# openjamoses/TOSEM-2021-Replication

Measured on AMD Instinct MI355X. Metric: train_tokens_per_s, higher is better.
Workload: dtype bf16; 1 GPU; model=mltc-base, global_batch=128, seq_len=512, parallelism=dp1

## Files before the change

csrc/flash_attn.hip:

```cpp

#include "common.h"
#include "launchers.h"
#include "philox.h"

typedef __attribute__((ext_vector_type(16))) float f32x16;
typedef __attribute__((ext_vector_type(2))) unsigned uint2_t;
typedef __attribute__((ext_vector_type(4))) unsigned uint4_t;

#define FA_DH 64
#define FA_KVB 32
#define FA_QB 32
#define FA_WAVES 4
#define FA_BLOCK (FA_WAVES * WAVE)
#define FA_QWG (FA_WAVES * FA_QB)
#define FA_Q2WG (2 * FA_QWG)

#define TILE_LDS_BYTES (FA_KVB * 128)
#define FWD_LDS_BYTES (2 * TILE_LDS_BYTES + FA_WAVES * 64 * sizeof(float))
#define BWD_LDS_BYTES (2 * TILE_LDS_BYTES + 64 * sizeof(float))
#define BWD_SEG_LDS_BYTES (BWD_LDS_BYTES + 32 * sizeof(int))
#define DQ_LDS_BYTES TILE_LDS_BYTES
#define DQR_LDS_BYTES (2 * TILE_LDS_BYTES + 16)
#define FA_DQR_WAVES(drop) ((drop) ? 1 : 2)

struct FaGeom {
  long qkv_bs, qkv_hs; int qkv_rs;
  long o_bs, o_hs; int o_rs;
  static FaGeom bhld(int H, int L) {
    return {(long)H * L * FA_DH, (long)L * FA_DH, FA_DH,
            (long)H * L * FA_DH, (long)L * FA_DH, FA_DH};
  }
  static FaGeom packed(int H, int L) {
    const int D = H * FA_DH;
    return {(long)L * 3 * D, 64L, 3 * D, (long)L * D, 64L, D};
  }
};


__device__ __forceinline__ int kswz(int row, int byte_off) {
  return byte_off ^ ((row & 7) << 4);
}

__device__ __forceinline__ int c_row(int r, int half) {
  return (r & 3) + 8 * (r >> 2) + 4 * half;
}

struct FaStager {
  int row, byte;
  __device__ __forceinline__ explicit FaStager(int tid)
      : row(tid >> 3), byte((tid & 7) * 16) {}
  __device__ __forceinline__ short8_t load(const short* base, int row0,
                                           int rs) const {
    return *(const short8_t*)(base + (long)(row0 + row) * rs + (byte >> 1));
  }
  __device__ __forceinline__ void store(short* lds, short8_t v) const {
    *(short8_t*)((char*)lds + row * 128 + kswz(row, byte)) = v;
  }
};

__device__ __forceinline__ short8_t tile_row_frag(const short* lds, int col,
                                                  int half, int c) {
  return *(const short8_t*)((const char*)lds + col * 128 +
                            kswz(col, (16 * c + 8 * half) * 2));
}

__device__ __forceinline__ void cvt_pk_swap(const float (&s)[16], int r0,
                                            int r1, uint4_t& u, int i) {
  unsigned lo, hi;
  asm("v_cvt_pk_bf16_f32 %0, %1, %2\n\ts_nop 1" : "=v"(lo)
      : "v"(s[r0]), "v"(s[r0 + 1]));
  asm("v_cvt_pk_bf16_f32 %0, %1, %2\n\ts_nop 1" : "=v"(hi)
      : "v"(s[r1]), "v"(s[r1 + 1]));
  auto sw = __builtin_amdgcn_permlane32_swap(lo, hi, false, false);
  u[i] = sw[0]; u[i + 2] = sw[1];
}

__device__ __forceinline__ void c_to_afrag2(const float (&sa)[16],
                                            short8_t (&fa)[2],
                                            const float (&sb)[16],
                                            short8_t (&fb)[2]) {
#pragma unroll
  for (int c = 0; c < 2; ++c) {
    uint4_t ua, ub;
#pragma unroll
    for (int i = 0; i < 2; ++i) {
      int r0 = c * 8 + 2 * i;
      int r1 = c * 8 + 4 + 2 * i;
      cvt_pk_swap(sa, r0, r1, ua, i);
      cvt_pk_swap(sb, r0, r1, ub, i);
    }
    fa[c] = __builtin_bit_cast(short8_t, ua);
    fb[c] = __builtin_bit_cast(short8_t, ub);
  }
}

struct FaTrFrags {
  uint2_t r[8];
  __device__ __forceinline__ short8_t frag(int c, int t) const {
    uint4_t w;
    w[0] = r[c * 4 + 0 * 2 + t][0];
    w[1] = r[c * 4 + 0 * 2 + t][1];
    w[2] = r[c * 4 + 1 * 2 + t][0];
    w[3] = r[c * 4 + 1 * 2 + t][1];
    return __builtin_bit_cast(short8_t, w);
  }
};

struct FaTrOffsets { unsigned a[8]; };

__device__ __forceinline__ FaTrOffsets tr_offsets(int lane, int half) {
  const int row_mate = (lane >> 2) & 3;
  const int d_lane = 16 * ((lane >> 4) & 1) + 4 * (lane & 3);
  FaTrOffsets o;
#pragma unroll
  for (int c = 0; c < 2; ++c)
#pragma unroll
    for (int rr = 0; rr < 2; ++rr)
#pragma unroll
      for (int t = 0; t < 2; ++t) {
        int row = 16 * c + 8 * half + 4 * rr + row_mate;
        int dcol = (32 * t + d_lane) * 2;
        o.a[c * 4 + rr * 2 + t] = row * 128 + kswz(row, dcol);
      }
  return o;
}

__device__ __forceinline__ void tr_issue(const short* lds,
                                         const FaTrOffsets& o, FaTrFrags& f) {
  const unsigned base = (unsigned)(unsigned long)(char*)lds;
  unsigned a[8];
#pragma unroll
  for (int i = 0; i < 8; ++i) a[i] = base + o.a[i];
  asm volatile(
      "ds_read_b64_tr_b16 %0, %8\n\t"
      "ds_read_b64_tr_b16 %1, %9\n\t"
      "ds_read_b64_tr_b16 %2, %10\n\t"
      "ds_read_b64_tr_b16 %3, %11\n\t"
      "ds_read_b64_tr_b16 %4, %12\n\t"
      "ds_read_b64_tr_b16 %5, %13\n\t"
      "ds_read_b64_tr_b16 %6, %14\n\t"
      "ds_read_b64_tr_b16 %7, %15\n\t"
      "s_waitcnt lgkmcnt(0)"
      : "=&v"(f.r[0]), "=&v"(f.r[1]), "=&v"(f.r[2]), "=&v"(f.r[3]),
        "=&v"(f.r[4]), "=&v"(f.r[5]), "=&v"(f.r[6]), "=&v"(f.r[7])
      : "v"(a[0]), "v"(a[1]), "v"(a[2]), "v"(a[3]), "v"(a[4]), "v"(a[5]),
        "v"(a[6]), "v"(a[7])
      : "memory");
}

__device__ __forceinline__ void tr_gather(const short* lds,
                                          const FaTrOffsets& o, FaTrFrags& f) {
  tr_issue(lds, o, f);
  __builtin_amdgcn_sched_barrier(0);
}

struct FaQBlocks { int bh, qA, qB; };

__device__ __forceinline__ FaQBlocks fa_qblocks(int L, int wid) {
  const int n_qblocks = (L + FA_Q2WG - 1) / FA_Q2WG;
  const int bid = xcd_group_remap(blockIdx.x, gridDim.x, n_qblocks);
  const int qA = (bid % n_qblocks) * FA_Q2WG + wid * FA_QB;
  return {bid / n_qblocks, qA, qA + FA_QWG};
}

__device__ __forceinline__ float fa_half_merge(float s) {
  return s + __shfl_xor(s, 32, WAVE);
}

__device__ __forceinline__ void fa_colsum_merge_store(const float* cs, int tid,
                                                      float* dst0,
                                                      float* dst1) {
  if (tid < 2 * FA_DH) {
    const int slot = tid / FA_DH, c = tid % FA_DH;
    const float* p = cs + slot * FA_WAVES * FA_DH + c;
    float s = p[0];
#pragma unroll
    for (int w = 1; w < FA_WAVES; ++w) s += p[w * FA_DH];
    float* dst = slot ? dst1 : dst0;
    if (dst) dst[c] = s;
  }
}

__device__ __forceinline__ int fa_last_active_kv(const float* mrow, int L,
                                                 int tid, int* scratch) {
  if (tid == 0) *scratch = -1;
  __syncthreads();
  int loc = -1;
  for (int kv = tid; kv < L; kv += FA_BLOCK)
    if (mrow[kv] > -1.0e8f) loc = kv;
  if (loc >= 0) atomicMax(scratch, loc);
  __syncthreads();
  return *scratch;
}

#define FA_SEG_BIAS -1.0e9f

struct FaRange { int lo, hi; };

__device__ __forceinline__ FaRange fa_seg_range(const int* srow, int L,
                                                int r_lo, int r_hi, int tid,
                                                int* scratch) {
  const int s_first = srow[r_lo], s_last = srow[r_hi];
  if (tid == 0) { scratch[0] = r_lo; scratch[1] = r_hi; }
  __syncthreads();
  int lo = r_lo, hi = r_hi;
  for (int j = tid; j < L; j += FA_BLOCK) {
    const int s = srow[j];
    if (s == s_first) lo = min(lo, j);
    if (s == s_last) hi = max(hi, j);
  }
  atomicMin(&scratch[0], lo);
  atomicMax(&scratch[1], hi);
  __syncthreads();
  return {scratch[0], scratch[1]};
}

__device__ __forceinline__ bool fa_seg_tile_live(const int (&r)[16], int a,
                                                 int b) {
  bool hit = false;
#pragma unroll
  for (int i = 0; i < 16; ++i) hit |= (r[i] == a) | (r[i] == b);
  return __builtin_amdgcn_ballot_w64(hit) != 0;
}

__device__ __forceinline__ unsigned long long fa_live_window(
    const unsigned char* dead_bh, int t0, int n_t, int lane) {
  const int t = t0 + lane;
  bool lv = t < n_t;
  if (lv && dead_bh) lv = dead_bh[t] == 0;
  return __builtin_amdgcn_ballot_w64(lv);
}

__device__ __forceinline__ void fa_store_zero_tile(short* base, int rs, int q0,
                                                   int L, int lane) {
#pragma unroll
  for (int i = 0; i < 4; ++i) {
    const int row = q0 + 8 * i + (lane >> 3);
    if (row < L)
      *(short8_t*)(base + (long)row * rs + (lane & 7) * 8) = (short8_t)(0);
  }
}

struct FaLiveScan {
  const unsigned char* dead_bh;
  int n_t, lane, win;
  unsigned long long bits;
  __device__ __forceinline__ FaLiveScan(const unsigned char* d, int n_t_,
                                        int lane_)
      : dead_bh(d), n_t(n_t_), lane(lane_), win(-1), bits(0) {}
  __device__ __forceinline__ void preload() {
    if (dead_bh) { win = 0; bits = fa_live_window(dead_bh, 0, n_t, lane); }
  }
  __device__ __forceinline__ int next(int qt, int n_q) {
    if (!dead_bh) return qt;
    while (qt < n_q) {
      if ((qt >> 6) != win) {
        win = qt >> 6;
        bits = fa_live_window(dead_bh, win << 6, n_t, lane);
      }
      const unsigned long long m = bits >> (qt & 63);
      if (m) return min(qt + (int)__builtin_ctzll(m), n_q);
      qt = (win + 1) << 6;
    }
    return n_q;
  }
};

#ifndef FA_DROP_QUAD_SHARE
#define FA_DROP_QUAD_SHARE 1
#endif

template <int G>
__device__ __forceinline__ unsigned fa_quad_bcast(unsigned v) {
  return (unsigned)__builtin_amdgcn_mov_dpp((int)v, G * 0x55, 0xf, 0xf, true);
}

template <int G>
__device__ __forceinline__ unsigned fa_drop_group_kvreg(const unsigned (&w)[4],
                                                        int i, unsigned thr) {
  const unsigned t0 = fa_quad_bcast<G>(w[0]), t1 = fa_quad_bcast<G>(w[1]);
  const unsigned t2 = fa_quad_bcast<G>(w[2]), t3 = fa_quad_bcast<G>(w[3]);
  const unsigned word = i == 0 ? t0 : i == 1 ? t1 : i == 2 ? t2 : t3;
  unsigned m = 0;
#pragma unroll
  for (int j = 0; j < 4; ++j)
    m |= (((word >> (8 * j)) & 0xffu) >= thr ? 1u : 0u) << (4 * G + j);
  return m;
}

__device__ __forceinline__ unsigned fa_drop_keep16_kvreg(
    const FaDrop& dr, unsigned long long rowblk, int kblk0, int lane) {
  const int i = lane & 3;
  unsigned w[4];
#if FA_DROP_QUAD_SHARE
  fa_drop_block(dr, rowblk + (unsigned)(kblk0 + 2 * i), w);
  return fa_drop_group_kvreg<0>(w, i, dr.thr) |
         fa_drop_group_kvreg<1>(w, i, dr.thr) |
         fa_drop_group_kvreg<2>(w, i, dr.thr) |
         fa_drop_group_kvreg<3>(w, i, dr.thr);
#else
  unsigned m = 0;
#pragma unroll
  for (int g = 0; g < 4; ++g) {
    fa_drop_block(dr, rowblk + (unsigned)(kblk0 + 2 * g), w);
    const unsigned word = i == 0 ? w[0] : i == 1 ? w[1] : i == 2 ? w[2] : w[3];
#pragma unroll
    for (int j = 0; j < 4; ++j)
      m |= (((word >> (8 * j)) & 0xffu) >= dr.thr ? 1u : 0u) << (4 * g + j);
  }
  return m;
#endif
}

template <int G>
__device__ __forceinline__ unsigned fa_drop_group_qreg(const unsigned (&w)[4],
                                                       int sh, unsigned thr) {
  unsigned m = 0;
#pragma unroll
  for (int j = 0; j < 4; ++j)
    m |= (((fa_quad_bcast<G>(w[j]) >> sh) & 0xffu) >= thr ? 1u : 0u)
         << (4 * G + j);
  return m;
}

__device__ __forceinline__ unsigned fa_drop_keep16_qreg(
    const FaDrop& dr, unsigned long long colblk, unsigned nb, int qblk0,
    int lane) {
  const int i = lane & 3;
  unsigned w[4];
#if FA_DROP_QUAD_SHARE
  fa_drop_block(dr, colblk + (unsigned long long)(qblk0 + 2 * i) * nb, w);
  return fa_drop_group_qreg<0>(w, 8 * i, dr.thr) |
         fa_drop_group_qreg<1>(w, 8 * i, dr.thr) |
         fa_drop_group_qreg<2>(w, 8 * i, dr.thr) |
         fa_drop_group_qreg<3>(w, 8 * i, dr.thr);
#else
  unsigned m = 0;
#pragma unroll
  for (int g = 0; g < 4; ++g) {
    fa_drop_block(dr, colblk + (unsigned long long)(qblk0 + 2 * g) * nb, w);
#pragma unroll
    for (int j = 0; j < 4; ++j)
      m |= (((w[j] >> (8 * i)) & 0xffu) >= dr.thr ? 1u : 0u) << (4 * g + j);
  }
  return m;
#endif
}

template <bool SEG, bool DROP>
__global__ void __launch_bounds__(FA_BLOCK, 2)
flash_fwd_kernel(const short* __restrict__ q, const short* __restrict__ k,
                 const short* __restrict__ v, const float* __restrict__ mask,
                 const int* __restrict__ seg,
                 short* __restrict__ o, float* __restrict__ lse,
                 int B, int H, int L, float scale, FaGeom g, FaDrop dr) {
  extern __shared__ __attribute__((aligned(16))) char smem[];
  short* k_lds = (short*)smem;
  short* v_lds = (short*)(smem + TILE_LDS_BYTES);
  float* alpha_lds = (float*)(smem + 2 * TILE_LDS_BYTES);

  const int tid = threadIdx.x;
  const int lane = tid & (WAVE - 1);
  const int wid = tid / WAVE;
  const int col = lane & 31;
  const int half = lane >> 5;
  const FaTrOffsets tro = tr_offsets(lane, half);

  const FaQBlocks qb = fa_qblocks(L, wid);
  const int b = qb.bh / H;
  const int h = qb.bh % H;
  const long qkv_off = (long)b * g.qkv_bs + (long)h * g.qkv_hs;
  const long o_off = (long)b * g.o_bs + (long)h * g.o_hs;
  const int my_qA = qb.qA + col;
  const int my_qB = qb.qB + col;
  const bool validA = my_qA < L;
  const bool validB = my_qB < L;
  const float* mrow = (!SEG && mask) ? mask + (long)b * L : nullptr;
  const int* srow = SEG ? seg + (long)b * L : nullptr;
  int sqA = 0, sqB = 0;
  if constexpr (SEG) {
    sqA = srow[validA ? my_qA : L - 1];
    sqB = srow[validB ? my_qB : L - 1];
  }

  short8_t qfA[4], qfB[4];
  {
    const short* qrA = q + qkv_off + (long)(validA ? my_qA : L - 1) * g.qkv_rs;
    const short* qrB = q + qkv_off + (long)(validB ? my_qB : L - 1) * g.qkv_rs;
#pragma unroll
    for (int c = 0; c < 4; ++c) {
      qfA[c] = *(const short8_t*)(qrA + c * 16 + half * 8);
      qfB[c] = *(const short8_t*)(qrB + c * 16 + half * 8);
    }
  }

  f32x16 oA[2], oB[2];
#pragma unroll
  for (int t = 0; t < 2; ++t) { oA[t] = (f32x16)(0.f); oB[t] = (f32x16)(0.f); }
  float mA = -3.0e38f, lA = 0.f, mB = -3.0e38f, lB = 0.f;
  unsigned long long dblkA = 0, dblkB = 0;
  if constexpr (DROP) {
    const unsigned long long nb = (unsigned)L / 4;
    dblkA = ((unsigned long long)qb.bh * nb + (unsigned)(my_qA >> 2)) * nb;
    dblkB = ((unsigned long long)qb.bh * nb + (unsigned)(my_qB >> 2)) * nb;
  }

  const int n_kv = L / FA_KVB;
  int kt_begin = 0;
  int n_kv_eff = n_kv;
  if (mrow) {
    int last = fa_last_active_kv(mrow, L, tid, (int*)alpha_lds);
    if (last >= 0) n_kv_eff = min(n_kv, last / FA_KVB + 1);
  }
  if constexpr (SEG) {
    const int q_lo = qb.qA - wid * FA_QB;
    const FaRange kr = fa_seg_range(srow, L, q_lo, min(q_lo + FA_Q2WG, L) - 1,
                                    tid, (int*)alpha_lds);
    kt_begin = kr.lo / FA_KVB;
    n_kv_eff = kr.hi / FA_KVB + 1;
  }
  const FaStager st(tid);
  short8_t kv8 = st.load(k + qkv_off, kt_begin * FA_KVB, g.qkv_rs);
  short8_t vv8 = st.load(v + qkv_off, kt_begin * FA_KVB, g.qkv_rs);
  for (int kt = kt_begin; kt < n_kv_eff; ++kt) {
    const int kv0 = kt * FA_KVB;
    __syncthreads();
    st.store(k_lds, kv8);
    st.store(v_lds, vv8);
    __syncthreads();
    if (kt + 1 < n_kv_eff) {
      kv8 = st.load(k + qkv_off, kv0 + FA_KVB, g.qkv_rs);
      vv8 = st.load(v + qkv_off, kv0 + FA_KVB, g.qkv_rs);
    }

    float mb_r[16];
    int sk_r[16];
#pragma unroll
    for (int r = 0; r < 16; ++r) {
      if constexpr (SEG) sk_r[r] = srow[kv0 + c_row(r, half)];
      else mb_r[r] = mrow ? mrow[kv0 + c_row(r, half)] : 0.f;
    }
    if constexpr (SEG) {
      if (!fa_seg_tile_live(sk_r, sqA, sqB)) continue;
    }

    f32x16 sA = (f32x16)(0.f), sB = (f32x16)(0.f);
    __builtin_amdgcn_s_setprio(1);
#pragma unroll
    for (int c = 0; c < 4; ++c) {
      short8_t kf = tile_row_frag(k_lds, col, half, c);
      sA = __builtin_amdgcn_mfma_f32_32x32x16_bf16(kf, qfA[c], sA, 0, 0, 0);
      sB = __builtin_amdgcn_mfma_f32_32x32x16_bf16(kf, qfB[c], sB, 0, 0, 0);
    }
    __builtin_amdgcn_s_setprio(0);

    float svA[16], svB[16];
    float tmaxA = -3.0e38f, tmaxB = -3.0e38f;
#pragma unroll
    for (int r = 0; r < 16; ++r) {
      float mbA, mbB;
      if constexpr (SEG) {
        mbA = sk_r[r] == sqA ? 0.f : FA_SEG_BIAS;
        mbB = sk_r[r] == sqB ? 0.f : FA_SEG_BIAS;
      } else {
        mbA = mbB = mb_r[r];
      }
      float xA = sA[r] * scale + mbA;
      float xB = sB[r] * scale + mbB;
      svA[r] = xA; svB[r] = xB;
      tmaxA = fmaxf(tmaxA, xA);
      tmaxB = fmaxf(tmaxB, xB);
    }
    tmaxA = fmaxf(tmaxA, __shfl_xor(tmaxA, 32, WAVE));
    tmaxB = fmaxf(tmaxB, __shfl_xor(tmaxB, 32, WAVE));
    float mnA = fmaxf(mA, tmaxA), mnB = fmaxf(mB, tmaxB);
    float aA = __expf(mA - mnA), aB = __expf(mB - mnB);
    float rsA = 0.f, rsB = 0.f;
#pragma unroll
    for (int r = 0; r < 16; ++r) {
      svA[r] = __expf(svA[r] - mnA);
      svB[r] = __expf(svB[r] - mnB);
      rsA += svA[r];
      rsB += svB[r];
    }
    rsA += __shfl_xor(rsA, 32, WAVE);
    rsB += __shfl_xor(rsB, 32, WAVE);
    lA = lA * aA + rsA; mA = mnA;
    lB = lB * aB + rsB; mB = mnB;

    if (__builtin_amdgcn_ballot_w64(aA != 1.f || aB != 1.f)) {
      alpha_lds[wid * 64 + col] = aA;
      alpha_lds[wid * 64 + 32 + col] = aB;
#pragma unroll
      for (int t = 0; t < 2; ++t) {
#pragma unroll
        for (int r = 0; r < 16; ++r) {
          int qrow = c_row(r, half);
          oA[t][r] *= alpha_lds[wid * 64 + qrow];
          oB[t][r] *= alpha_lds[wid * 64 + 32 + qrow];
        }
      }
    }

    if constexpr (DROP) {
      const unsigned keepA =
          fa_drop_keep16_kvreg(dr, dblkA, kv0 / 4 + half, lane);
      const unsigned keepB =
          fa_drop_keep16_kvreg(dr, dblkB, kv0 / 4 + half, lane);
#pragma unroll
      for (int r = 0; r < 16; ++r) {
        if (!((keepA >> r) & 1u)) svA[r] = 0.f;
        if (!((keepB >> r) & 1u)) svB[r] = 0.f;
      }
    }

    short8_t pfA[2], pfB[2];
    c_to_afrag2(svA, pfA, svB, pfB);

    FaTrFrags vT;
    tr_gather(v_lds, tro, vT);
    __builtin_amdgcn_s_setprio(1);
#pragma unroll
    for (int t = 0; t < 2; ++t) {
#pragma unroll
      for (int c = 0; c < 2; ++c) {
        short8_t vf = vT.frag(c, t);
        oA[t] = __builtin_amdgcn_mfma_f32_32x32x16_bf16(pfA[c], vf, oA[t],
                                                        0, 0, 0);
        oB[t] = __builtin_amdgcn_mfma_f32_32x32x16_bf16(pfB[c], vf, oB[t],
                                                        0, 0, 0);
      }
    }
    __builtin_amdgcn_s_setprio(0);
  }

  if (lse != nullptr && half == 0) {
    if (validA) lse[(long)qb.bh * L + my_qA] = mA + __logf(lA);
    if (validB) lse[(long)qb.bh * L + my_qB] = mB + __logf(lB);
  }
  const float one = DROP ? dr.scale : 1.0f;
  const float invA = one / lA, invB = one / lB;
#pragma unroll
  for (int r = 0; r < 16; ++r) {
    int rloc = c_row(r, half);
    float iA = __shfl(invA, rloc, WAVE);
    float iB = __shfl(invB, rloc, WAVE);
    int qA = qb.qA + rloc, qB = qb.qB + rloc;
#pragma unroll
    for (int t = 0; t < 2; ++t) {
      if (qA < L)
        o[o_off + (long)qA * g.o_rs + 32 * t + col] =
            f32_to_bf16(oA[t][r] * iA);
      if (qB < L)
        o[o_off + (long)qB * g.o_rs + 32 * t + col] =
            f32_to_bf16(oB[t][r] * iB);
    }
  }
}

static int fa_row_blocks(int B, int L, int rows_per_wg) {
  return B * ((L + rows_per_wg - 1) / rows_per_wg);
}
static dim3 fa_grid(int B, int H, int L, int rows_per_wg) {
  return dim3(H * fa_row_blocks(B, L, rows_per_wg));
}

extern "C" int flash_bias_ws_rows(int B, int L) {
  return fa_row_blocks(B, L, FA_QWG);
}

static void fa_fwd_dispatch(const short* q, const short* k, const short* v,
                            const void* mask, const void* seg, void* o,
                            void* lse, int B, int H, int L, float scale,
                            FaGeom g, FaDrop dr, hipStream_t stream) {
  const dim3 grid = fa_grid(B, H, L, FA_Q2WG);
#define FA_FWD_SEG_ARGS                                                       \
  q, k, v, nullptr, (const int*)seg, (short*)o, (float*)lse, B, H, L, scale,  \
      g, dr
#define FA_FWD_ARGS                                                           \
  q, k, v, (const float*)mask, nullptr, (short*)o, (float*)lse, B, H, L,      \
      scale, g, dr
  if (seg && dr.thr)
    flash_fwd_kernel<true, true><<<grid, FA_BLOCK, FWD_LDS_BYTES, stream>>>(
        FA_FWD_SEG_ARGS);
  else if (seg)
    flash_fwd_kernel<true, false><<<grid, FA_BLOCK, FWD_LDS_BYTES, stream>>>(
        FA_FWD_SEG_ARGS);
  else if (dr.thr)
    flash_fwd_kernel<false, true><<<grid, FA_BLOCK, FWD_LDS_BYTES, stream>>>(
        FA_FWD_ARGS);
  else
    flash_fwd_kernel<false, false><<<grid, FA_BLOCK, FWD_LDS_BYTES, stream>>>(
        FA_FWD_ARGS);
#undef FA_FWD_ARGS
#undef FA_FWD_SEG_ARGS
}

static bool fa_drop_ok(unsigned thr) { return thr <= 255u; }

extern "C" hipError_t flash_fwd_launch(const void* q, const void* k,
                                       const void* v, const void* mask,
                                       const void* seg, void* o, void* lse,
                                       int B, int H, int L, float scale,
                                       unsigned long long drop_seed,
                                       unsigned drop_call, unsigned drop_site,
                                       unsigned drop_thr,
                                       hipStream_t stream) {
  if (!fa_drop_ok(drop_thr)) return hipErrorInvalidValue;
  fa_fwd_dispatch((const short*)q, (const short*)k, (const short*)v, mask,
                  seg, o, lse, B, H, L, scale, FaGeom::bhld(H, L),
                  fa_drop_make(drop_seed, drop_call, drop_site, drop_thr),
                  stream);
  return hipGetLastError();
}

extern "C" hipError_t flash_fwd_packed_launch(const void* qkv,
                                              const void* mask,
                                              const void* seg, void* o,
                                              void* lse, int B, int H, int L,
                                              float scale,
                                              unsigned long long drop_seed,
                                              unsigned drop_call,
                                              unsigned drop_site,
                                              unsigned drop_thr,
                                              hipStream_t stream) {
  if (!fa_drop_ok(drop_thr)) return hipErrorInvalidValue;
  const int D = H * FA_DH;
  fa_fwd_dispatch((const short*)qkv, (const short*)qkv + D,
                  (const short*)qkv + 2 * D, mask, seg, o, lse, B, H, L,
                  scale, FaGeom::packed(H, L),
                  fa_drop_make(drop_seed, drop_call, drop_site, drop_thr),
                  stream);
  return hipGetLastError();
}




template <bool SEG, bool BIAS, bool DROP>
__global__ void __launch_bounds__(FA_BLOCK, 2)
flash_bwd_fused_kernel(const short* __restrict__ q, const short* __restrict__ k,
                       const short* __restrict__ v,
                       const short* __restrict__ dout,
                       const float* __restrict__ mask,
                       const int* __restrict__ seg,
                       const float* __restrict__ lse,
                       const float* __restrict__ ddot,
                       const unsigned char* __restrict__ dead,
                       short* __restrict__ ds, short* __restrict__ dk,
                       short* __restrict__ dv,
                       int B, int H, int L, float scale, FaGeom g,
                       float* __restrict__ bias_ws, int bias_ld, FaDrop dr) {
  extern __shared__ __attribute__((aligned(16))) char smem[];
  short* q_lds = (short*)smem;
  short* do_lds = (short*)(smem + TILE_LDS_BYTES);
  float* lse_lds = (float*)(smem + 2 * TILE_LDS_BYTES);
  float* dd_lds = lse_lds + 32;
  int* seg_lds = (int*)(dd_lds + 32);

  const int tid = threadIdx.x;
  const int lane = tid & (WAVE - 1);
  const int wid = tid / WAVE;
  const int col = lane & 31;
  const int half = lane >> 5;
  const FaTrOffsets tro = tr_offsets(lane, half);

  const int n_kvblocks = (L + FA_QWG - 1) / FA_QWG;
  int bid = xcd_group_remap(blockIdx.x, gridDim.x, n_kvblocks);
  int bh = bid / n_kvblocks;
  int kb = bid % n_kvblocks;
  const int b = bh / H;
  const int h = bh % H;
  const long qkv_off = (long)b * g.qkv_bs + (long)h * g.qkv_hs;
  const long o_off = (long)b * g.o_bs + (long)h * g.o_hs;
  const long bh_sq = (long)bh * L * L;
  const int kv_base = kb * FA_QWG + wid * FA_KVB;
  const int my_kv = kv_base + col;
  const bool kv_valid = my_kv < L;
  const float* mrow = (!SEG && mask) ? mask + (long)b * L : nullptr;
  const float mb = mrow ? mrow[min(my_kv, L - 1)] : 0.f;
  const int* srow = SEG ? seg + (long)b * L : nullptr;
  int sk = 0;
  if constexpr (SEG) sk = srow[min(my_kv, L - 1)];
  const unsigned drop_nb = (unsigned)L / 4;
  unsigned long long dblk = 0;
  if constexpr (DROP)
    dblk = (unsigned long long)bh * drop_nb * drop_nb +
           (unsigned)(min(my_kv, L - 1) >> 2);

  FaLiveScan live(ds == nullptr && dead ? dead + (long)bh * (L / 32) : nullptr,
                  L / 32, lane);
  live.preload();

  bool skip_tile = false;
  bool wave_skip = false;
  if (mrow && ds == nullptr) {
    int* any_lds = (int*)lse_lds;
    if (tid == 0) *any_lds = 0;
    __syncthreads();
    if (kv_valid && mb > -1.0e8f) *any_lds = 1;
    __syncthreads();
    skip_tile = (*any_lds == 0) && (mrow[0] > -1.0e8f);
    __syncthreads();
    wave_skip = !skip_tile && (mrow[0] > -1.0e8f) &&
        __builtin_amdgcn_ballot_w64(kv_valid && mb > -1.0e8f) == 0;
  }

  short8_t kf[4], vf[4];
  if (!skip_tile) {
    const short* kr = k + qkv_off + (long)(kv_valid ? my_kv : L - 1) * g.qkv_rs;
// ... 175 lines not shown
    flash_bwd_fused_kernel<false, false, true>
        <<<grid, FA_BLOCK, BWD_LDS_BYTES, stream>>>(FA_BWD_ARGS);
  } else if (seg && bias_ws) {
    flash_bwd_fused_kernel<true, true, false>
        <<<grid, FA_BLOCK, BWD_SEG_LDS_BYTES, stream>>>(FA_BWD_SEG_ARGS);
  } else if (seg) {
    flash_bwd_fused_kernel<true, false, false>
        <<<grid, FA_BLOCK, BWD_SEG_LDS_BYTES, stream>>>(FA_BWD_SEG_ARGS);
  } else if (bias_ws) {
    flash_bwd_fused_kernel<false, true, false>
        <<<grid, FA_BLOCK, BWD_LDS_BYTES, stream>>>(FA_BWD_ARGS);
  } else {
    flash_bwd_fused_kernel<false, false, false>
        <<<grid, FA_BLOCK, BWD_LDS_BYTES, stream>>>(FA_BWD_ARGS);
  }
#undef FA_BWD_ARGS
#undef FA_BWD_SEG_ARGS
}

extern "C" hipError_t flash_bwd_fused_launch(
    const void* q, const void* k, const void* v, const void* dout,
    const void* mask, const void* seg, const void* lse, const void* ddot,
    const void* dead, void* ds, void* dk, void* dv, int B, int H, int L,
    float scale, unsigned long long drop_seed, unsigned drop_call,
    unsigned drop_site, unsigned drop_thr, hipStream_t stream) {
  if ((seg || drop_thr) && ds) return hipErrorInvalidValue;
  if (!fa_drop_ok(drop_thr)) return hipErrorInvalidValue;
  fa_bwd_fused_dispatch((const short*)q, (const short*)k, (const short*)v,
                        dout, mask, seg, lse, ddot, dead, ds, (short*)dk,
                        (short*)dv, B, H, L, scale, FaGeom::bhld(H, L),
                        nullptr,
                        fa_drop_make(drop_seed, drop_call, drop_site, drop_thr),
                        stream);
  return hipGetLastError();
}

extern "C" hipError_t flash_bwd_fused_packed_launch(
    const void* qkv, const void* dout, const void* mask, const void* seg,
    const void* lse, const void* ddot, const void* dead, void* dqkv,
    void* bias_ws, int B, int H, int L, float scale,
    unsigned long long drop_seed, unsigned drop_call, unsigned drop_site,
    unsigned drop_thr, hipStream_t stream) {
  if (drop_thr && bias_ws) return hipErrorInvalidValue;
  if (!fa_drop_ok(drop_thr)) return hipErrorInvalidValue;
  const int D = H * FA_DH;
  fa_bwd_fused_dispatch((const short*)qkv, (const short*)qkv + D,
                        (const short*)qkv + 2 * D, dout, mask, seg, lse, ddot,
                        dead, nullptr, (short*)dqkv + D, (short*)dqkv + 2 * D, B, H,
                        L, scale, FaGeom::packed(H, L), (float*)bias_ws,
                        fa_drop_make(drop_seed, drop_call, drop_site, drop_thr),
                        stream);
  return hipGetLastError();
}

extern "C" __global__ void __launch_bounds__(FA_BLOCK, 2)
flash_dq_kernel(const short* __restrict__ ds, const short* __restrict__ k,
                short* __restrict__ dq, int B, int H, int L) {
  extern __shared__ __attribute__((aligned(16))) char smem[];
  short* k_lds = (short*)smem;

  const int tid = threadIdx.x;
  const int lane = tid & (WAVE - 1);
  const int wid = tid / WAVE;
  const int col = lane & 31;
  const int half = lane >> 5;
  const FaTrOffsets tro = tr_offsets(lane, half);

  const FaQBlocks qb = fa_qblocks(L, wid);
  const long bh_off = (long)qb.bh * L * FA_DH;
  const long bh_sq = (long)qb.bh * L * L;
  const int my_qA = min(qb.qA + col, L - 1);
  const int my_qB = min(qb.qB + col, L - 1);
  const short* dsA_row = ds + bh_sq + (long)my_qA * L;
  const short* dsB_row = ds + bh_sq + (long)my_qB * L;

  f32x16 oA[2], oB[2];
#pragma unroll
  for (int t = 0; t < 2; ++t) { oA[t] = (f32x16)(0.f); oB[t] = (f32x16)(0.f); }

  const int n_kv = L / FA_KVB;
  const FaStager st(tid);
  short8_t kv8 = st.load(k + bh_off, 0, FA_DH);
  for (int kt = 0; kt < n_kv; ++kt) {
    const int kv0 = kt * FA_KVB;
    __syncthreads();
    st.store(k_lds, kv8);
    __syncthreads();
    if (kt + 1 < n_kv) kv8 = st.load(k + bh_off, kv0 + FA_KVB, FA_DH);
    short8_t aA[2], aB[2];
#pragma unroll
    for (int c = 0; c < 2; ++c) {
      aA[c] = *(const short8_t*)(dsA_row + kv0 + 16 * c + 8 * half);
      aB[c] = *(const short8_t*)(dsB_row + kv0 + 16 * c + 8 * half);
    }
    FaTrFrags kT;
    tr_gather(k_lds, tro, kT);
    __builtin_amdgcn_s_setprio(1);
#pragma unroll
    for (int t = 0; t < 2; ++t) {
#pragma unroll
      for (int c = 0; c < 2; ++c) {
        short8_t kf = kT.frag(c, t);
        oA[t] = __builtin_amdgcn_mfma_f32_32x32x16_bf16(aA[c], kf, oA[t],
                                                        0, 0, 0);
        oB[t] = __builtin_amdgcn_mfma_f32_32x32x16_bf16(aB[c], kf, oB[t],
                                                        0, 0, 0);
      }
    }
    __builtin_amdgcn_s_setprio(0);
  }

#pragma unroll
  for (int t = 0; t < 2; ++t) {
#pragma unroll
    for (int r = 0; r < 16; ++r) {
      int rloc = c_row(r, half);
      int qA = qb.qA + rloc, qB = qb.qB + rloc;
      if (qA < L)
        dq[bh_off + (long)qA * FA_DH + 32 * t + col] = f32_to_bf16(oA[t][r]);
      if (qB < L)
        dq[bh_off + (long)qB * FA_DH + 32 * t + col] = f32_to_bf16(oB[t][r]);
    }
  }
}

extern "C" hipError_t flash_dq_launch(const void* ds, const void* k, void* dq,
                                      int B, int H, int L,
                                      hipStream_t stream) {
  flash_dq_kernel<<<fa_grid(B, H, L, FA_Q2WG), FA_BLOCK, DQ_LDS_BYTES,
                    stream>>>(
      (const short*)ds, (const short*)k, (short*)dq, B, H, L);
  return hipGetLastError();
}

template <bool SEG, bool BIAS, bool DROP>
__global__ void __launch_bounds__(FA_BLOCK, FA_DQR_WAVES(DROP))
flash_dq_recompute_kernel(const short* __restrict__ q,
                          const short* __restrict__ k,
                          const short* __restrict__ v,
                          const short* __restrict__ dout,
                          const float* __restrict__ mask,
                          const int* __restrict__ seg,
                          const float* __restrict__ lse,
                          const float* __restrict__ ddot,
                          const unsigned char* __restrict__ dead,
                          short* __restrict__ dq,
                          int B, int H, int L, float scale, FaGeom g,
                          float* __restrict__ bias_ws, int bias_ld,
                          FaDrop dr) {
  extern __shared__ __attribute__((aligned(16))) char smem[];
  short* k_lds = (short*)smem;
  short* v_lds = (short*)(smem + TILE_LDS_BYTES);
  int* skip_scratch = (int*)(smem + 2 * TILE_LDS_BYTES);

  const int tid = threadIdx.x;
  const int lane = tid & (WAVE - 1);
  const int wid = tid / WAVE;
  const int col = lane & 31;
  const int half = lane >> 5;
  const FaTrOffsets tro = tr_offsets(lane, half);

  const FaQBlocks qb = fa_qblocks(L, wid);
  const int b = qb.bh / H;
  const int h = qb.bh % H;
  const long qkv_off = (long)b * g.qkv_bs + (long)h * g.qkv_hs;
  const long o_off = (long)b * g.o_bs + (long)h * g.o_hs;

  bool tile_dead = false;
  if (dead) {
    const int n_t = L / FA_QB;
    const int t = (qb.qA - wid * FA_QB) / FA_QB + lane;
    tile_dead = lane < 8 && (t >= n_t || dead[(long)qb.bh * n_t + t] != 0);
  }

  const int my_qA = qb.qA + col;
  const int my_qB = qb.qB + col;
  const bool validA = my_qA < L;
  const bool validB = my_qB < L;
  const float* mrow = (!SEG && mask) ? mask + (long)b * L : nullptr;
  const int* srow = SEG ? seg + (long)b * L : nullptr;
  int sqA = 0, sqB = 0;
  if constexpr (SEG) {
    sqA = srow[validA ? my_qA : L - 1];
    sqB = srow[validB ? my_qB : L - 1];
  }

  short8_t qfA[4], qfB[4], dofA[4], dofB[4];
  {
    const short* qrA = q + qkv_off + (long)(validA ? my_qA : L - 1) * g.qkv_rs;
    const short* qrB = q + qkv_off + (long)(validB ? my_qB : L - 1) * g.qkv_rs;
    const short* drA = dout + o_off + (long)(validA ? my_qA : L - 1) * g.o_rs;
    const short* drB = dout + o_off + (long)(validB ? my_qB : L - 1) * g.o_rs;
#pragma unroll
    for (int c = 0; c < 4; ++c) {
      qfA[c] = *(const short8_t*)(qrA + c * 16 + half * 8);
      qfB[c] = *(const short8_t*)(qrB + c * 16 + half * 8);
      dofA[c] = *(const short8_t*)(drA + c * 16 + half * 8);
      dofB[c] = *(const short8_t*)(drB + c * 16 + half * 8);
    }
  }
  const float lseA = lse[(long)qb.bh * L + (validA ? my_qA : L - 1)];
  const float lseB = lse[(long)qb.bh * L + (validB ? my_qB : L - 1)];
  const float ddA = ddot[(long)qb.bh * L + (validA ? my_qA : L - 1)];
  const float ddB = ddot[(long)qb.bh * L + (validB ? my_qB : L - 1)];
  unsigned long long dblkA = 0, dblkB = 0;
  if constexpr (DROP) {
    const unsigned long long nb = (unsigned)L / 4;
    dblkA = ((unsigned long long)qb.bh * nb + (unsigned)(my_qA >> 2)) * nb;
    dblkB = ((unsigned long long)qb.bh * nb + (unsigned)(my_qB >> 2)) * nb;
  }

  const unsigned dmask = (unsigned)__builtin_amdgcn_ballot_w64(tile_dead);
  if (dmask == 0xffu) {
    fa_store_zero_tile(dq + qkv_off, g.qkv_rs, qb.qA, L, lane);
    fa_store_zero_tile(dq + qkv_off, g.qkv_rs, qb.qB, L, lane);
    if constexpr (BIAS) {
      if (tid < 2 * FA_DH) {
        const int n128 = (L + FA_QWG - 1) / FA_QWG;
        const int blk = (qb.qA - wid * FA_QB) / FA_QWG + tid / FA_DH;
        if (blk < n128)
          bias_ws[((long)b * n128 + blk) * bias_ld + h * FA_DH + tid % FA_DH] =
              0.f;
      }
    }
    return;
  }
  const bool wave_dead = ((dmask >> wid) & 0x11u) == 0x11u;

  f32x16 dqA[2], dqB[2];
#pragma unroll
  for (int t = 0; t < 2; ++t) { dqA[t] = (f32x16)(0.f); dqB[t] = (f32x16)(0.f); }

  const int n_kv = L / FA_KVB;
  int kt_begin = 0;
  int n_kv_eff = n_kv;
  if (mrow) {
    int last = fa_last_active_kv(mrow, L, tid, skip_scratch);
    if (last >= 0) n_kv_eff = min(n_kv, last / FA_KVB + 1);
  }
  if constexpr (SEG) {
    const int q_lo = qb.qA - wid * FA_QB;
    const FaRange kr = fa_seg_range(srow, L, q_lo, min(q_lo + FA_Q2WG, L) - 1,
                                    tid, skip_scratch);
    kt_begin = kr.lo / FA_KVB;
    n_kv_eff = kr.hi / FA_KVB + 1;
  }
  const FaStager st(tid);
  short8_t kv8 = st.load(k + qkv_off, kt_begin * FA_KVB, g.qkv_rs);
  short8_t vv8 = st.load(v + qkv_off, kt_begin * FA_KVB, g.qkv_rs);
  for (int kt = kt_begin; kt < n_kv_eff; ++kt) {
    const int kv0 = kt * FA_KVB;
    __syncthreads();
    st.store(k_lds, kv8);
    st.store(v_lds, vv8);
    __syncthreads();
    if (kt + 1 < n_kv_eff) {
      kv8 = st.load(k + qkv_off, kv0 + FA_KVB, g.qkv_rs);
      vv8 = st.load(v + qkv_off, kv0 + FA_KVB, g.qkv_rs);
    }
    if (wave_dead) continue;

    float mb_r[16];
    int sk_r[16];
#pragma unroll
    for (int r = 0; r < 16; ++r) {
      if constexpr (SEG) sk_r[r] = srow[kv0 + c_row(r, half)];
      else mb_r[r] = mrow ? mrow[kv0 + c_row(r, half)] : 0.f;
    }
    if constexpr (SEG) {
      if (!fa_seg_tile_live(sk_r, sqA, sqB)) continue;
    }

    f32x16 sA = (f32x16)(0.f), sB = (f32x16)(0.f);
    f32x16 pA = (f32x16)(0.f), pB = (f32x16)(0.f);
    __builtin_amdgcn_s_setprio(1);
#pragma unroll
    for (int c = 0; c < 4; ++c) {
      short8_t kf = tile_row_frag(k_lds, col, half, c);
      short8_t vf = tile_row_frag(v_lds, col, half, c);
      sA = __builtin_amdgcn_mfma_f32_32x32x16_bf16(kf, qfA[c], sA, 0, 0, 0);
      sB = __builtin_amdgcn_mfma_f32_32x32x16_bf16(kf, qfB[c], sB, 0, 0, 0);
      pA = __builtin_amdgcn_mfma_f32_32x32x16_bf16(vf, dofA[c], pA, 0, 0, 0);
      pB = __builtin_amdgcn_mfma_f32_32x32x16_bf16(vf, dofB[c], pB, 0, 0, 0);
    }
    __builtin_amdgcn_s_setprio(0);

    float gA[16], gB[16];
    unsigned keepA = 0, keepB = 0;
    if constexpr (DROP) {
      keepA = fa_drop_keep16_kvreg(dr, dblkA, kv0 / 4 + half, lane);
      keepB = fa_drop_keep16_kvreg(dr, dblkB, kv0 / 4 + half, lane);
    }
#pragma unroll
    for (int r = 0; r < 16; ++r) {
      float mbA, mbB;
      if constexpr (SEG) {
        mbA = sk_r[r] == sqA ? 0.f : FA_SEG_BIAS;
        mbB = sk_r[r] == sqB ? 0.f : FA_SEG_BIAS;
      } else {
        mbA = mbB = mb_r[r];
      }
      float expA = __expf(sA[r] * scale + mbA - lseA);
      float expB = __expf(sB[r] * scale + mbB - lseB);
      float dpA = pA[r], dpB = pB[r];
      if constexpr (DROP) {
        dpA = (keepA >> r) & 1u ? dpA * dr.scale : 0.f;
        dpB = (keepB >> r) & 1u ? dpB * dr.scale : 0.f;
      }
      gA[r] = scale * expA * (dpA - ddA);
      gB[r] = scale * expB * (dpB - ddB);
    }

    short8_t gfA[2], gfB[2];
    c_to_afrag2(gA, gfA, gB, gfB);

    FaTrFrags kT;
    tr_gather(k_lds, tro, kT);
    __builtin_amdgcn_s_setprio(1);
#pragma unroll
    for (int t = 0; t < 2; ++t) {
#pragma unroll
      for (int c = 0; c < 2; ++c) {
        short8_t kf = kT.frag(c, t);
        dqA[t] = __builtin_amdgcn_mfma_f32_32x32x16_bf16(gfA[c], kf, dqA[t],
                                                         0, 0, 0);
        dqB[t] = __builtin_amdgcn_mfma_f32_32x32x16_bf16(gfB[c], kf, dqB[t],
                                                         0, 0, 0);
      }
    }
    __builtin_amdgcn_s_setprio(0);
  }

  float csA[2] = {0.f, 0.f}, csB[2] = {0.f, 0.f};
#pragma unroll
  for (int t = 0; t < 2; ++t) {
#pragma unroll
    for (int r = 0; r < 16; ++r) {
      int rloc = c_row(r, half);
      int qA = qb.qA + rloc, qB = qb.qB + rloc;
      if (qA < L) {
        const short a16 = f32_to_bf16(dqA[t][r]);
        dq[qkv_off + (long)qA * g.qkv_rs + 32 * t + col] = a16;
        if constexpr (BIAS) csA[t] += bf16_to_f32(a16);
      }
      if (qB < L) {
        const short b16 = f32_to_bf16(dqB[t][r]);
        dq[qkv_off + (long)qB * g.qkv_rs + 32 * t + col] = b16;
        if constexpr (BIAS) csB[t] += bf16_to_f32(b16);
      }
    }
  }
  if constexpr (BIAS) {
    float* cs = (float*)smem;
    __syncthreads();
#pragma unroll
    for (int t = 0; t < 2; ++t) {
      float sA_ = fa_half_merge(csA[t]);
      float sB_ = fa_half_merge(csB[t]);
      if (half == 0) {
        cs[(0 * FA_WAVES + wid) * FA_DH + 32 * t + col] = sA_;
        cs[(1 * FA_WAVES + wid) * FA_DH + 32 * t + col] = sB_;
      }
    }
    __syncthreads();
    const int n128 = (L + FA_QWG - 1) / FA_QWG;
    const int blkA = (qb.qA - wid * FA_QB) / FA_QWG;
    float* row = bias_ws + ((long)b * n128 + blkA) * bias_ld + h * FA_DH;
    fa_colsum_merge_store(cs, tid, row,
                          blkA + 1 < n128 ? row + bias_ld : nullptr);
  }
}

static void fa_dq_recompute_dispatch(const short* q, const short* k,
                                     const short* v, const void* dout,
                                     const void* mask, const void* seg,
                                     const void* lse, const void* ddot,
                                     const void* dead, void* dq, int B, int H,
                                     int L, float scale, FaGeom g,
                                     float* bias_ws, FaDrop dr,
                                     hipStream_t stream) {
  const dim3 grid = fa_grid(B, H, L, FA_Q2WG);
  const int bias_ld = 3 * H * FA_DH;
#define FA_DQR_SEG_ARGS                                                       \
  q, k, v, (const short*)dout, nullptr, (const int*)seg, (const float*)lse,   \
      (const float*)ddot, (const unsigned char*)dead, (short*)dq, B, H, L,    \
      scale, g, bias_ws, bias_ld, dr
#define FA_DQR_ARGS                                                           \
  q, k, v, (const short*)dout, (const float*)mask, nullptr,                   \
      (const float*)lse, (const float*)ddot, (const unsigned char*)dead,      \
      (short*)dq, B, H, L, scale, g, bias_ws, bias_ld, dr
  if (seg && dr.thr) {
    flash_dq_recompute_kernel<true, false, true>
        <<<grid, FA_BLOCK, DQR_LDS_BYTES, stream>>>(FA_DQR_SEG_ARGS);
  } else if (dr.thr) {
    flash_dq_recompute_kernel<false, false, true>
        <<<grid, FA_BLOCK, DQR_LDS_BYTES, stream>>>(FA_DQR_ARGS);
  } else if (seg && bias_ws) {
    flash_dq_recompute_kernel<true, true, false>
        <<<grid, FA_BLOCK, DQR_LDS_BYTES, stream>>>(FA_DQR_SEG_ARGS);
  } else if (seg) {
    flash_dq_recompute_kernel<true, false, false>
        <<<grid, FA_BLOCK, DQR_LDS_BYTES, stream>>>(FA_DQR_SEG_ARGS);
  } else if (bias_ws) {
    flash_dq_recompute_kernel<false, true, false>
        <<<grid, FA_BLOCK, DQR_LDS_BYTES, stream>>>(FA_DQR_ARGS);
  } else {
    flash_dq_recompute_kernel<false, false, false>
        <<<grid, FA_BLOCK, DQR_LDS_BYTES, stream>>>(FA_DQR_ARGS);
  }
#undef FA_DQR_ARGS
#undef FA_DQR_SEG_ARGS
}

extern "C" hipError_t flash_dq_recompute_launch(
    const void* q, const void* k, const void* v, const void* dout,
    const void* mask, const void* seg, const void* lse, const void* ddot,
    const void* dead, void* dq, int B, int H, int L, float scale,
    unsigned long long drop_seed, unsigned drop_call, unsigned drop_site,
    unsigned drop_thr, hipStream_t stream) {
  if (!fa_drop_ok(drop_thr)) return hipErrorInvalidValue;
  fa_dq_recompute_dispatch((const short*)q, (const short*)k, (const short*)v,
                           dout, mask, seg, lse, ddot, dead, dq, B, H, L, scale,
                           FaGeom::bhld(H, L), nullptr,
                           fa_drop_make(drop_seed, drop_call, drop_site,
                                        drop_thr),
                           stream);
  return hipGetLastError();
}

extern "C" hipError_t flash_dq_recompute_packed_launch(
    const void* qkv, const void* dout, const void* mask, const void* seg,
    const void* lse, const void* ddot, const void* dead, void* dqkv,
    void* bias_ws, int B, int H, int L, float scale,
    unsigned long long drop_seed, unsigned drop_call, unsigned drop_site,
    unsigned drop_thr, hipStream_t stream) {
  if (drop_thr && bias_ws) return hipErrorInvalidValue;
  if (!fa_drop_ok(drop_thr)) return hipErrorInvalidValue;
  const int D = H * FA_DH;
  fa_dq_recompute_dispatch((const short*)qkv, (const short*)qkv + D,
                           (const short*)qkv + 2 * D, dout, mask, seg, lse,
                           ddot, dead, dqkv, B, H, L, scale,
                           FaGeom::packed(H, L), (float*)bias_ws,
                           fa_drop_make(drop_seed, drop_call, drop_site,
                                        drop_thr),
                           stream);
  return hipGetLastError();
}

__device__ __forceinline__ float fa_row_dot(short4_t a, short4_t c) {
  float s = 0.f;
#pragma unroll
  for (int j = 0; j < 4; ++j) s += bf16_to_f32(a[j]) * bf16_to_f32(c[j]);
#pragma unroll
  for (int off = 8; off > 0; off >>= 1) s += __shfl_xor(s, off, 16);
  return s;
}

__device__ __forceinline__ void fa_dot_tile(const short* dr, const short* orow,
                                            long rs, float* dd,
                                            unsigned char* dead_flag,
                                            int n_valid, int lane) {
  const int sub = lane & 15, grp = lane >> 4;
  short4_t a[8], c[8];
#pragma unroll
  for (int p = 0; p < 8; ++p) {
    const int r = min(4 * p + grp, n_valid - 1);
    a[p] = *(const short4_t*)(dr + r * rs + sub * 4);
    c[p] = *(const short4_t*)(orow + r * rs + sub * 4);
  }
  unsigned nz = 0;
#pragma unroll
  for (int p = 0; p < 8; ++p) {
    const int r = 4 * p + grp;
    const float s = fa_row_dot(a[p], c[p]);
    if (r < n_valid) {
#pragma unroll
      for (int j = 0; j < 4; ++j) nz |= (unsigned)a[p][j] & 0x7fffu;
      if (sub == 0) dd[r] = s;
    }
  }
  const bool live = __builtin_amdgcn_ballot_w64(nz != 0) != 0;
  if (lane == 0) *dead_flag = live ? 0 : 1;
}

extern "C" __global__ void __launch_bounds__(FA_BLOCK)
fa_dot_kernel(const short* __restrict__ dout, const short* __restrict__ o,
              float* __restrict__ ddot, unsigned char* __restrict__ dead,
              long n_rows) {
  const long tile = (long)blockIdx.x * FA_WAVES + threadIdx.x / WAVE;
  const long row0 = tile * FA_QB;
  if (row0 >= n_rows) return;
  fa_dot_tile(dout + row0 * FA_DH, o + row0 * FA_DH, FA_DH, ddot + row0,
              dead + tile, (int)min((long)FA_QB, n_rows - row0),
              threadIdx.x & (WAVE - 1));
}

extern "C" __global__ void __launch_bounds__(FA_BLOCK)
fa_dot_packed_kernel(const short* __restrict__ dout,
                     const short* __restrict__ o, float* __restrict__ ddot,
                     unsigned char* __restrict__ dead, int B, int H, int L) {
  const int D = H * FA_DH;
  const int n_t = L / FA_QB;
  const long wv = (long)blockIdx.x * FA_WAVES + threadIdx.x / WAVE;
  if (wv >= (long)B * n_t * H) return;
// ... 74 lines not shown
```

Measured before the change: 811,300 tokens/s.

## Stage attention outputs through LDS for coalesced stores, vectorize mask loads, prefetch KV earlier

The forward and dQ-reduce epilogues now write bf16 results into a per-wave swizzled LDS staging tile and then emit 16-byte row-contiguous global stores, replacing scattered 2-byte stores. Mask and segment-id reads are vectorized into int4/float4 loads. In the non-segment path the first K/V tile load is issued before the mask scan so it overlaps with that scan. The cost is extra LDS per block (staging for each wave), which could reduce occupancy under the two-blocks-per-CU launch bound.

```diff
diff --git a/csrc/flash_attn.hip b/csrc/flash_attn.hip
--- a/csrc/flash_attn.hip
+++ b/csrc/flash_attn.hip
@@ -16,11 +16,14 @@
 #define FA_Q2WG (2 * FA_QWG)
 
 #define TILE_LDS_BYTES (FA_KVB * 128)
-#define FWD_LDS_BYTES (2 * TILE_LDS_BYTES + FA_WAVES * 64 * sizeof(float))
+#define OUT_LDS_BYTES (FA_WAVES * 2 * TILE_LDS_BYTES)
+#define FWD_TILES_BYTES (2 * TILE_LDS_BYTES + FA_WAVES * 64 * sizeof(float))
+#define DQR_TILES_BYTES (2 * TILE_LDS_BYTES + 16)
+#define FWD_LDS_BYTES (FWD_TILES_BYTES + OUT_LDS_BYTES)
 #define BWD_LDS_BYTES (2 * TILE_LDS_BYTES + 64 * sizeof(float))
 #define BWD_SEG_LDS_BYTES (BWD_LDS_BYTES + 32 * sizeof(int))
 #define DQ_LDS_BYTES TILE_LDS_BYTES
-#define DQR_LDS_BYTES (2 * TILE_LDS_BYTES + 16)
+#define DQR_LDS_BYTES (DQR_TILES_BYTES + OUT_LDS_BYTES)
 #define FA_DQR_WAVES(drop) ((drop) ? 1 : 2)
 
 struct FaGeom {
@@ -154,6 +157,26 @@
   __builtin_amdgcn_sched_barrier(0);
 }
 
+template <bool SEG>
+__device__ __forceinline__ void fa_load_kv_rows(const void* row, int kv0,
+                                                int half, int (&sk_r)[16],
+                                                float (&mb_r)[16]) {
+#pragma unroll
+  for (int j = 0; j < 4; ++j) {
+    const int kv = kv0 + 8 * j + 4 * half;
+    if constexpr (SEG) {
+      const int4 s4 = *(const int4*)((const int*)row + kv);
+      sk_r[4 * j] = s4.x; sk_r[4 * j + 1] = s4.y;
+      sk_r[4 * j + 2] = s4.z; sk_r[4 * j + 3] = s4.w;
+    } else {
+      const float4 m4 = row ? *(const float4*)((const float*)row + kv)
+                            : make_float4(0.f, 0.f, 0.f, 0.f);
+      mb_r[4 * j] = m4.x; mb_r[4 * j + 1] = m4.y;
+      mb_r[4 * j + 2] = m4.z; mb_r[4 * j + 3] = m4.w;
+    }
+  }
+}
+
 struct FaQBlocks { int bh, qA, qB; };
 
 __device__ __forceinline__ FaQBlocks fa_qblocks(int L, int wid) {
@@ -238,6 +261,42 @@
     const int row = q0 + 8 * i + (lane >> 3);
     if (row < L)
       *(short8_t*)(base + (long)row * rs + (lane & 7) * 8) = (short8_t)(0);
+  }
+}
+
+__device__ __forceinline__ short* fa_out_stage(char* out_lds, int wid,
+                                               int slot) {
+  return (short*)(out_lds + (wid * 2 + slot) * TILE_LDS_BYTES);
+}
+
+__device__ __forceinline__ void fa_store_tile_rows(short* stage,
+                                                   const short (&v)[2][16],
+                                                   short* base, int rs,
+                                                   int row0, int L, int lane) {
+  if (row0 >= L) return;
+  const int col = lane & 31, half = lane >> 5;
+#pragma unroll
+  for (int t = 0; t < 2; ++t) {
+#pragma unroll
+    for (int r = 0; r < 16; ++r) {
+      const int row = c_row(r, half);
+      *(short*)((char*)stage + row * 128 + kswz(row, (32 * t + col) * 2)) =
+          v[t][r];
+    }
+  }
+  __builtin_amdgcn_fence(__ATOMIC_ACQ_REL, "wavefront");
+  __builtin_amdgcn_wave_barrier();
+  short8_t w[4];
+#pragma unroll
+  for (int i = 0; i < 4; ++i) {
+    const int row = 8 * i + (lane >> 3);
+    w[i] = *(const short8_t*)((const char*)stage + row * 128 +
+                              kswz(row, (lane & 7) * 16));
+  }
+#pragma unroll
+  for (int i = 0; i < 4; ++i) {
+    const int row = row0 + 8 * i + (lane >> 3);
+    if (row < L) *(short8_t*)(base + (long)row * rs + (lane & 7) * 8) = w[i];
   }
 }
 
@@ -358,6 +417,7 @@
   short* k_lds = (short*)smem;
   short* v_lds = (short*)(smem + TILE_LDS_BYTES);
   float* alpha_lds = (float*)(smem + 2 * TILE_LDS_BYTES);
+  char* out_lds = smem + FWD_TILES_BYTES;
 
   const int tid = threadIdx.x;
   const int lane = tid & (WAVE - 1);
@@ -408,6 +468,12 @@
   const int n_kv = L / FA_KVB;
   int kt_begin = 0;
   int n_kv_eff = n_kv;
+  const FaStager st(tid);
+  short8_t kv8, vv8;
+  if constexpr (!SEG) {
+    kv8 = st.load(k + qkv_off, 0, g.qkv_rs);
+    vv8 = st.load(v + qkv_off, 0, g.qkv_rs);
+  }
   if (mrow) {
     int last = fa_last_active_kv(mrow, L, tid, (int*)alpha_lds);
     if (last >= 0) n_kv_eff = min(n_kv, last / FA_KVB + 1);
@@ -419,9 +485,10 @@
     kt_begin = kr.lo / FA_KVB;
     n_kv_eff = kr.hi / FA_KVB + 1;
   }
-  const FaStager st(tid);
-  short8_t kv8 = st.load(k + qkv_off, kt_begin * FA_KVB, g.qkv_rs);
-  short8_t vv8 = st.load(v + qkv_off, kt_begin * FA_KVB, g.qkv_rs);
+  if constexpr (SEG) {
+    kv8 = st.load(k + qkv_off, kt_begin * FA_KVB, g.qkv_rs);
+    vv8 = st.load(v + qkv_off, kt_begin * FA_KVB, g.qkv_rs);
+  }
   for (int kt = kt_begin; kt < n_kv_eff; ++kt) {
     const int kv0 = kt * FA_KVB;
     __syncthreads();
@@ -435,11 +502,8 @@
 
     float mb_r[16];
     int sk_r[16];
-#pragma unroll
-    for (int r = 0; r < 16; ++r) {
-      if constexpr (SEG) sk_r[r] = srow[kv0 + c_row(r, half)];
-      else mb_r[r] = mrow ? mrow[kv0 + c_row(r, half)] : 0.f;
-    }
+    fa_load_kv_rows<SEG>(SEG ? (const void*)srow : (const void*)mrow, kv0, half,
+                         sk_r, mb_r);
     if constexpr (SEG) {
       if (!fa_seg_tile_live(sk_r, sqA, sqB)) continue;
     }
@@ -540,22 +604,22 @@
   }
   const float one = DROP ? dr.scale : 1.0f;
   const float invA = one / lA, invB = one / lB;
+  short a16[2][16], b16[2][16];
 #pragma unroll
   for (int r = 0; r < 16; ++r) {
     int rloc = c_row(r, half);
     float iA = __shfl(invA, rloc, WAVE);
     float iB = __shfl(invB, rloc, WAVE);
-    int qA = qb.qA + rloc, qB = qb.qB + rloc;
 #pragma unroll
     for (int t = 0; t < 2; ++t) {
-      if (qA < L)
-        o[o_off + (long)qA * g.o_rs + 32 * t + col] =
-            f32_to_bf16(oA[t][r] * iA);
-      if (qB < L)
-        o[o_off + (long)qB * g.o_rs + 32 * t + col] =
-            f32_to_bf16(oB[t][r] * iB);
-    }
-  }
+      a16[t][r] = f32_to_bf16(oA[t][r] * iA);
+      b16[t][r] = f32_to_bf16(oB[t][r] * iB);
+    }
+  }
+  fa_store_tile_rows(fa_out_stage(out_lds, wid, 0), a16, o + o_off, g.o_rs,
+                     qb.qA, L, lane);
+  fa_store_tile_rows(fa_out_stage(out_lds, wid, 1), b16, o + o_off, g.o_rs,
+                     qb.qB, L, lane);
 }
 
 static int fa_row_blocks(int B, int L, int rows_per_wg) {
@@ -1037,6 +1101,7 @@
   short* k_lds = (short*)smem;
   short* v_lds = (short*)(smem + TILE_LDS_BYTES);
   int* skip_scratch = (int*)(smem + 2 * TILE_LDS_BYTES);
+  char* out_lds = smem + DQR_TILES_BYTES;
 
   const int tid = threadIdx.x;
   const int lane = tid & (WAVE - 1);
@@ -1119,6 +1184,12 @@
   const int n_kv = L / FA_KVB;
   int kt_begin = 0;
   int n_kv_eff = n_kv;
+  const FaStager st(tid);
+  short8_t kv8, vv8;
+  if constexpr (!SEG) {
+    kv8 = st.load(k + qkv_off, 0, g.qkv_rs);
+    vv8 = st.load(v + qkv_off, 0, g.qkv_rs);
+  }
   if (mrow) {
     int last = fa_last_active_kv(mrow, L, tid, skip_scratch);
     if (last >= 0) n_kv_eff = min(n_kv, last / FA_KVB + 1);
@@ -1130,9 +1201,10 @@
     kt_begin = kr.lo / FA_KVB;
     n_kv_eff = kr.hi / FA_KVB + 1;
   }
-  const FaStager st(tid);
-  short8_t kv8 = st.load(k + qkv_off, kt_begin * FA_KVB, g.qkv_rs);
-  short8_t vv8 = st.load(v + qkv_off, kt_begin * FA_KVB, g.qkv_rs);
+  if constexpr (SEG) {
+    kv8 = st.load(k + qkv_off, kt_begin * FA_KVB, g.qkv_rs);
+    vv8 = st.load(v + qkv_off, kt_begin * FA_KVB, g.qkv_rs);
+  }
   for (int kt = kt_begin; kt < n_kv_eff; ++kt) {
     const int kv0 = kt * FA_KVB;
     __syncthreads();
@@ -1147,11 +1219,8 @@
 
     float mb_r[16];
     int sk_r[16];
-#pragma unroll
-    for (int r = 0; r < 16; ++r) {
-      if constexpr (SEG) sk_r[r] = srow[kv0 + c_row(r, half)];
-      else mb_r[r] = mrow ? mrow[kv0 + c_row(r, half)] : 0.f;
-    }
+    fa_load_kv_rows<SEG>(SEG ? (const void*)srow : (const void*)mrow, kv0, half,
+                         sk_r, mb_r);
     if constexpr (SEG) {
       if (!fa_seg_tile_live(sk_r, sqA, sqB)) continue;
     }
@@ -1217,24 +1286,24 @@
   }
 
   float csA[2] = {0.f, 0.f}, csB[2] = {0.f, 0.f};
+  short a16[2][16], b16[2][16];
 #pragma unroll
   for (int t = 0; t < 2; ++t) {
 #pragma unroll
     for (int r = 0; r < 16; ++r) {
-      int rloc = c_row(r, half);
-      int qA = qb.qA + rloc, qB = qb.qB + rloc;
-      if (qA < L) {
-        const short a16 = f32_to_bf16(dqA[t][r]);
-        dq[qkv_off + (long)qA * g.qkv_rs + 32 * t + col] = a16;
-        if constexpr (BIAS) csA[t] += bf16_to_f32(a16);
-      }
-      if (qB < L) {
-        const short b16 = f32_to_bf16(dqB[t][r]);
-        dq[qkv_off + (long)qB * g.qkv_rs + 32 * t + col] = b16;
-        if constexpr (BIAS) csB[t] += bf16_to_f32(b16);
-      }
-    }
-  }
+      a16[t][r] = f32_to_bf16(dqA[t][r]);
+      b16[t][r] = f32_to_bf16(dqB[t][r]);
+      if constexpr (BIAS) {
+        int rloc = c_row(r, half);
+        if (qb.qA + rloc < L) csA[t] += bf16_to_f32(a16[t][r]);
+        if (qb.qB + rloc < L) csB[t] += bf16_to_f32(b16[t][r]);
+      }
+    }
+  }
+  fa_store_tile_rows(fa_out_stage(out_lds, wid, 0), a16, dq + qkv_off,
+                     g.qkv_rs, qb.qA, L, lane);
+  fa_store_tile_rows(fa_out_stage(out_lds, wid, 1), b16, dq + qkv_off,
+                     g.qkv_rs, qb.qB, L, lane);
   if constexpr (BIAS) {
     float* cs = (float*)smem;
     __syncthreads();
```

Measured after the change: 820,100 tokens/s, median of 6. 1.1% higher.
